# jonassibbesen/rpvg

Measured on AMD Instinct MI355X. Metric: read-pairs quantified/sec, higher is better.
Workload: dtype f64

## Files before the change

### rpvg_amd/csrc/subset_em.hip

```cpp

#include "common.hpp"
#include "subset_pack.hpp"

#include <cmath>
#include <memory>

using namespace rpvg_hip_detail;

namespace {

constexpr uint32_t kMaxSelected = 1024;

struct MergedList {
    const uint32_t * a;
    const uint32_t * b;
    uint32_t na, nb, i, j;
    __device__ __forceinline__ MergedList(const uint32_t * a_in, uint32_t na_in, const uint32_t * b_in, uint32_t nb_in)
        : a(a_in), b(b_in), na(na_in), nb(nb_in), i(0), j(0) {}
    __device__ __forceinline__ bool done() const { return i >= na && j >= nb; }
    __device__ __forceinline__ uint32_t next() {
        if (j >= nb || (i < na && a[i] <= b[j])) return a[i++];
        return b[j++];
    }
};

struct Columns {
    const uint64_t * group_path_off;
    const uint32_t * group_path;
    uint64_t first_column;
    __device__ __forceinline__ MergedList list(const uint32_t first, const uint32_t second) const {
        const uint64_t a0 = group_path_off[first_column + first], a1 = group_path_off[first_column + first + 1];
        const uint64_t b0 = group_path_off[first_column + second], b1 = group_path_off[first_column + second + 1];
        return MergedList(group_path + a0, static_cast<uint32_t>(a1 - a0), group_path + b0, static_cast<uint32_t>(b1 - b0));
    }
};

__device__ __forceinline__ int compareLists(MergedList x, MergedList y) {
    while (!x.done() && !y.done()) {
        const uint32_t px = x.next(), py = y.next();
        if (px != py) return px < py ? -1 : 1;
    }
    if (x.done() && y.done()) return 0;
    return x.done() ? -1 : 1;
}

struct SelectArgs {
    uint32_t num_matrices;
    const uint32_t * pair_count;
    const uint64_t * pair_cap_off;
    const uint32_t * pair_first;
    const uint32_t * pair_second;
    const double * pair_value;
    const uint64_t * group_off;
    const uint64_t * group_path_off;
    const uint32_t * group_path;
    const uint32_t * cluster;
    const uint64_t * mat_rows;
    const uint64_t * cluster_row_off;
    const uint64_t * row_ent_off;
    const uint64_t * slot_off;
    double min_hap_prob;
    uint32_t segment_rows;
    uint32_t * slot_first;
    uint32_t * slot_second;
    double * slot_weight;
    uint32_t * slot_length;
    uint32_t * slot_columns;
    MatrixTotals * totals;
    SubsetHeader * header;
    uint32_t * big_matrices;
};

constexpr uint32_t kSmallSelected = 64;
constexpr uint32_t kSmallCachedPaths = 1024, kWideCachedPaths = 6144;

struct CachedColumns {
    const uint64_t * group_path_off;
    const uint32_t * paths;
    uint64_t first_column, base;
    __device__ __forceinline__ MergedList list(const uint32_t first, const uint32_t second) const {
        const uint64_t a0 = group_path_off[first_column + first], a1 = group_path_off[first_column + first + 1];
        const uint64_t b0 = group_path_off[first_column + second], b1 = group_path_off[first_column + second + 1];
        return MergedList(paths + (a0 - base), static_cast<uint32_t>(a1 - a0), paths + (b0 - base), static_cast<uint32_t>(b1 - b0));
    }
};

template <uint32_t CAP, uint32_t CACHE, int BLOCK>
__device__ __forceinline__ void selectSubsetsOfMatrix(const SelectArgs & args, const uint32_t m) {
    __shared__ uint32_t sel[CAP];
    __shared__ unsigned long long hash[CAP];
    __shared__ uint32_t length[CAP];
    __shared__ uint32_t leader[CAP];
    __shared__ double weight[CAP];
    __shared__ uint32_t order[CAP];
    __shared__ uint32_t cached_paths[CACHE];
    __shared__ uint32_t scratch[BLOCK / 64];
    __shared__ double sum_posterior;
    __shared__ unsigned long long red[3];
    __shared__ uint32_t n_retained;
    const uint32_t n_pairs = args.pair_count[m];
    const uint64_t base = args.pair_cap_off[m];
    const uint32_t * first = args.pair_first + base;
    const uint32_t * second = args.pair_second + base;
    const double * value = args.pair_value + base;
    const uint32_t k = args.cluster[m];
    MatrixTotals * out_totals = args.totals + m;
    const uint64_t col0 = args.group_off[m], col1 = args.group_off[m + 1];
    const uint64_t path0 = args.group_path_off[col0], path1 = args.group_path_off[col1];
    const bool cached = path1 - path0 <= CACHE;
    if (cached) {
        for (uint32_t i = threadIdx.x; i < path1 - path0; i += BLOCK) cached_paths[i] = args.group_path[path0 + i];
    }
    const CachedColumns columns{args.group_path_off, cached ? cached_paths : args.group_path, col0, cached ? path0 : 0};

    uint32_t n_sel = 0;
    for (uint32_t c = 0; c < n_pairs; c += BLOCK) {
        const uint32_t i = c + threadIdx.x;
        const uint32_t take = (i < n_pairs && value[i] >= args.min_hap_prob) ? 1u : 0u;
        uint32_t total;
        const uint32_t at = n_sel + blockExclusiveScan<BLOCK>(take, total, scratch);
        if (take && at < CAP) sel[at] = i;
        n_sel += total;
    }
    if (n_sel > CAP) {
        if (threadIdx.x == 0) {
            atomicAdd(&args.header->select_overflow, 1ull);
            *out_totals = MatrixTotals{0, 0, 0, 0, 0, 0};
        }
        return;
    }
    __syncthreads();
    if (threadIdx.x == 0) {
        double sum = 0;
        for (uint32_t s = 0; s < n_sel; ++s) sum += value[sel[s]];
        sum_posterior = sum;
        red[0] = red[1] = red[2] = 0;
        n_retained = 0;
    }
    for (uint32_t s = threadIdx.x; s < n_sel; s += BLOCK) {
        MergedList list = columns.list(first[sel[s]], second[sel[s]]);
        unsigned long long h = 1469598103934665603ull;
        uint32_t n = 0;
        while (!list.done()) {
            h = (h ^ list.next()) * 1099511628211ull;
            ++n;
        }
        hash[s] = h;
        length[s] = n;
    }
    __syncthreads();
    for (uint32_t s = threadIdx.x; s < n_sel; s += BLOCK) {
        uint32_t lead = s;
        for (uint32_t t = 0; t < s; ++t) {
            if (hash[t] == hash[s] && length[t] == length[s] &&
                compareLists(columns.list(first[sel[t]], second[sel[t]]), columns.list(first[sel[s]], second[sel[s]])) == 0) {
                lead = t;
                break;
            }
        }
        leader[s] = lead;
    }
    __syncthreads();
    for (uint32_t s = threadIdx.x; s < n_sel; s += BLOCK) {
        double w = 0;
        if (leader[s] == s) {
            for (uint32_t t = s; t < n_sel; ++t) {
                if (leader[t] == s) w += value[sel[t]];
            }
            w /= sum_posterior;
            if (w >= args.min_hap_prob) order[atomicAdd(&n_retained, 1u)] = s;
        }
        weight[s] = w;
    }
    __syncthreads();
    const uint32_t n_ret = n_retained;
    uint32_t padded = 1;
    while (padded < n_ret) padded <<= 1;
    for (uint32_t i = n_ret + threadIdx.x; i < padded; i += BLOCK) order[i] = 0xffffffffu;
    __syncthreads();
    auto before = [&](const uint32_t x, const uint32_t y) {
        if (x == 0xffffffffu) return false;
        if (y == 0xffffffffu) return true;
        return compareLists(columns.list(first[sel[x]], second[sel[x]]), columns.list(first[sel[y]], second[sel[y]])) < 0;
    };
    for (uint32_t size = 2; size <= padded; size <<= 1) {
        for (uint32_t stride = size >> 1; stride > 0; stride >>= 1) {
            for (uint32_t i = threadIdx.x; i < padded; i += BLOCK) {
                const uint32_t partner = i ^ stride;
                if (partner > i) {
                    const bool ascending = (i & size) == 0;
                    const uint32_t x = order[i], y = order[partner];
                    if (before(y, x) == ascending) {
                        order[i] = y;
                        order[partner] = x;
                    }
                }
            }
            __syncthreads();
        }
    }
    const uint64_t slot0 = args.slot_off[m];
    unsigned long long my_subsets = 0, my_length = 0, my_columns = 0;
    for (uint32_t rank = threadIdx.x; rank < n_ret; rank += BLOCK) {
        const uint32_t s = order[rank];
        uint32_t distinct = 0, previous = 0xffffffffu;
        MergedList walk = columns.list(first[sel[s]], second[sel[s]]);
        while (!walk.done()) {
            const uint32_t path = walk.next();
            distinct += (path != previous) ? 1u : 0u;
            previous = path;
        }
        args.slot_first[slot0 + rank] = first[sel[s]];
        args.slot_second[slot0 + rank] = second[sel[s]];
        args.slot_weight[slot0 + rank] = weight[s];
        args.slot_length[slot0 + rank] = length[s];
        args.slot_columns[slot0 + rank] = distinct;
        my_subsets += 1;
        my_length += length[s];
        my_columns += distinct;
    }
    if (my_subsets) {
        atomicAdd(&red[0], my_subsets);
        atomicAdd(&red[1], my_length);
        atomicAdd(&red[2], my_columns);
    }
    __syncthreads();
    if (threadIdx.x == 0) {
        const uint64_t r0 = args.cluster_row_off[k], r1 = args.cluster_row_off[k + 1];
        const unsigned long long rows = r1 - r0, entries = args.row_ent_off[r1] - args.row_ent_off[r0];
        *out_totals = MatrixTotals{red[0], red[1], red[2], red[0] * rows, red[0] * entries, red[0] * ((rows + args.segment_rows - 1) / args.segment_rows)};
    }
}

__global__ __launch_bounds__(64) void subsetSelectSmallKernel(const SelectArgs args) {
    const uint32_t m = blockIdx.x;
    if (m >= args.num_matrices) return;
    if (args.pair_count[m] > kSmallSelected) {
        if (threadIdx.x == 0) args.big_matrices[atomicAdd(&args.header->big_count, 1u)] = m;
        return;
    }
    selectSubsetsOfMatrix<kSmallSelected, kSmallCachedPaths, 64>(args, m);
}

__global__ __launch_bounds__(256) void subsetSelectWideKernel(const SelectArgs args) {
    const uint32_t count = args.header->big_count;
    for (uint32_t item = blockIdx.x; item < count; item += gridDim.x) {
        selectSubsetsOfMatrix<kMaxSelected, kWideCachedPaths, 256>(args, args.big_matrices[item]);
        __syncthreads();
    }
}

struct ExpandArgs {
    uint32_t num_matrices;
    const SubsetHeader * header;
    const MatrixTotals * totals;
    const MatrixTotals * bases;
    const uint64_t * slot_off;
    const uint32_t * slot_first;
    const uint32_t * slot_second;
    const double * slot_weight;
    const uint32_t * slot_length;
    const uint32_t * slot_columns;
    const uint64_t * group_off;
    const uint64_t * group_path_off;
    const uint32_t * group_path;
    const uint32_t * cluster;
    const uint64_t * cluster_row_off;
    const uint64_t * row_ent_off;
    uint32_t * sub_cluster;
    double * sub_weight;
    uint64_t * path_off;
    uint32_t * path;
    uint64_t * col_off;
    uint32_t * col_path;
    uint64_t * row_base;
    uint64_t * ent_base;
    uint64_t * seg_first;
    uint32_t * item_problem;
    uint32_t segment_rows;
    uint64_t * subset_off;
};

__global__ __launch_bounds__(256) void subsetExpandKernel(const ExpandArgs args) {
    constexpr int BLOCK = 256;
    __shared__ uint32_t scratch[BLOCK / 64];
    const uint32_t m = blockIdx.x;
    if (m >= args.num_matrices) return;
    const MatrixTotals base = args.bases[m];
    if (threadIdx.x == 0) {
        args.subset_off[m] = args.header->overflow ? 0 : base.subsets;
        if (m + 1 == args.num_matrices) args.subset_off[m + 1] = args.header->overflow ? 0 : args.header->subsets;
    }
    if (args.header->overflow) return;
    const uint32_t n = static_cast<uint32_t>(args.totals[m].subsets);
    const uint64_t slot0 = args.slot_off[m];
    const Columns columns{args.group_path_off, args.group_path, args.group_off[m]};
    const uint32_t k = args.cluster[m];
    const uint64_t r0 = args.cluster_row_off[k], r1 = args.cluster_row_off[k + 1];
    const uint64_t rows = r1 - r0, entries = args.row_ent_off[r1] - args.row_ent_off[r0];
    uint64_t length_run = base.list_length, columns_run = base.columns;
    for (uint32_t c = 0; c < n; c += BLOCK) {
        const uint32_t r = c + threadIdx.x;
        const uint32_t len = r < n ? args.slot_length[slot0 + r] : 0u, cols = r < n ? args.slot_columns[slot0 + r] : 0u;
        uint32_t len_total, cols_total;
        const uint32_t len_before = blockExclusiveScan<BLOCK>(len, len_total, scratch);
        const uint32_t cols_before = blockExclusiveScan<BLOCK>(cols, cols_total, scratch);
        if (r < n) {
            const uint64_t s = base.subsets + r;
            const uint64_t p0 = length_run + len_before, c0 = columns_run + cols_before;
            args.sub_cluster[s] = k;
            args.sub_weight[s] = args.slot_weight[slot0 + r];
            args.path_off[s] = p0;
            args.col_off[s] = c0;
            args.row_base[s] = base.rows + static_cast<uint64_t>(r) * rows;
            args.ent_base[s] = base.entries + static_cast<uint64_t>(r) * entries;
            const uint64_t segments = (rows + args.segment_rows - 1) / args.segment_rows, item0 = base.segments + static_cast<uint64_t>(r) * segments;
            args.seg_first[s] = item0;
            for (uint64_t item = item0; item < item0 + segments; ++item) args.item_problem[item] = static_cast<uint32_t>(s);
            MergedList list = columns.list(args.slot_first[slot0 + r], args.slot_second[slot0 + r]);
            uint32_t previous = 0xffffffffu;
            uint64_t pw = p0, cw = c0;
            while (!list.done()) {
                const uint32_t path = list.next();
                args.path[pw++] = path;
                if (path != previous) args.col_path[cw++] = path;
                previous = path;
            }
        }
        length_run += len_total;
        columns_run += cols_total;
    }
}

constexpr uint32_t kMergeLdsRecords = 2048;
constexpr unsigned long long kMergeNoRecord = ~0ull;
constexpr uint32_t kMergePathBits = 27, kMergeRankBits = 10;

struct MergeArgs {
    const SubsetHeader * header;
    uint32_t num_matrices;
    const uint64_t * subset_off;
    const double * weight;
    const uint64_t * path_off;
    const uint32_t * path;
    const uint64_t * col_off;
    const uint32_t * col_path;
    const double * abundances;
    const double * noise;
    const double * total;
    const uint32_t * cluster;
    const uint64_t * cluster_path_off;
    const uint32_t * path_group_id;
    unsigned long long * sort_key;
    uint32_t * sort_pos;
    double * rec_a0;
    double * rec_a1;
    uint32_t * merge_bad;
    unsigned char * packed;
};

__global__ __launch_bounds__(256) void subsetMergeKernel(const MergeArgs args) {
    constexpr int BLOCK = 256;
    __shared__ unsigned long long s_key[kMergeLdsRecords];
    __shared__ uint32_t s_pos[kMergeLdsRecords];
    __shared__ uint32_t s_scan[BLOCK / 64];
    const SubsetHeader h = *args.header;
    if (h.overflow) return;
    const uint32_t m = blockIdx.x, tid = threadIdx.x;
    const uint64_t M = args.num_matrices;
    if (m >= M) return;
    const PackedLayout lay = packedLayout(M, h.subsets, h.list_length, h.columns);
    uint32_t * set_count = reinterpret_cast<uint32_t *>(args.packed + lay.set_count);
    double * cluster_noise = reinterpret_cast<double *>(args.packed + lay.cluster_noise);
    uint32_t * set_first = reinterpret_cast<uint32_t *>(args.packed + lay.set_first);
    uint32_t * set_second = reinterpret_cast<uint32_t *>(args.packed + lay.set_second);
    double * set_posterior = reinterpret_cast<double *>(args.packed + lay.set_posterior);
    double * set_abund = reinterpret_cast<double *>(args.packed + lay.set_abund);
    const uint64_t s0 = args.subset_off[m];
    const uint32_t n = static_cast<uint32_t>(args.subset_off[m + 1] - s0);
    if (n == 0) {
        if (tid == 0) {
            set_count[m] = 0;
            cluster_noise[m] = 0.0;
        }
        return;
    }
    const uint64_t base = args.path_off[s0];
    const uint32_t Lm = static_cast<uint32_t>(args.path_off[s0 + n] - base);
    const uint32_t * gid = args.path_group_id + args.cluster_path_off[args.cluster[m]];
    if (tid == BLOCK - 1) {
        double noise = 0.0, sum_hap_prob = 0.0;
        for (uint32_t r = 0; r < n; ++r) {
            const double w = args.weight[s0 + r];
            sum_hap_prob = addRounded(sum_hap_prob, w);
            noise = addRounded(noise, mulRounded(args.noise[s0 + r], w));
        }
        cluster_noise[m] = addRounded(noise, mulRounded(addRounded(1.0, -sum_hap_prob), args.total[s0]));
    }
    uint32_t P2 = 2;
    while (P2 < Lm) P2 <<= 1;
    unsigned long long * keys = s_key;
    uint32_t * order = s_pos;
    if (P2 > kMergeLdsRecords) {
        keys = args.sort_key + 2 * base;
        order = args.sort_pos + 2 * base;
    }
    for (uint32_t pos = tid; pos < P2; pos += BLOCK) {
        unsigned long long key = kMergeNoRecord;
        if (pos < Lm) {
            uint32_t lo = 0, hi = n - 1;
            while (lo < hi) {
                const uint32_t mid = (lo + hi + 1) >> 1;
                if (args.path_off[s0 + mid] - base <= pos) lo = mid; else hi = mid - 1;
            }
            const uint32_t r = lo;
            const uint32_t l0 = static_cast<uint32_t>(args.path_off[s0 + r] - base), L = static_cast<uint32_t>(args.path_off[s0 + r + 1] - base) - l0;
            const uint32_t * list = args.path + base + l0;
            const uint32_t j = pos - l0;
            const uint32_t g = gid[list[j]];
            uint32_t members = 0, first = 0, second = 0;
            for (uint32_t t = 0; t < L; ++t) {
                if (gid[list[t]] == g) {
                    if (members == 0) first = t;
                    else if (members == 1) second = t;
                    ++members;
                }
            }
            if (members > 2) *args.merge_bad = 1;
            if (first == j && members <= 2) {
                const uint32_t p0 = list[first], p1 = (members == 2) ? list[second] : 0xffffffffu;
                const double w = args.weight[s0 + r];
                const uint64_t c0 = args.col_off[s0 + r];
                const uint32_t C = static_cast<uint32_t>(args.col_off[s0 + r + 1] - c0);
                const uint32_t * cols = args.col_path + c0;
                auto column = [&](const uint32_t p) {
                    uint32_t a = 0, b = C;
                    while (a < b) {
                        const uint32_t mid = (a + b) >> 1;
                        if (cols[mid] < p) a = mid + 1; else b = mid;
                    }
                    return a;
                };
                const double multiplicity = (members == 2 && p0 == p1) ? 2.0 : 1.0;
                args.rec_a0[base + pos] = mulRounded(args.abundances[c0 + column(p0)], w) / multiplicity;
                args.rec_a1[base + pos] = (members == 2) ? mulRounded(args.abundances[c0 + column(p1)], w) / multiplicity : 0.0;
                key = (static_cast<unsigned long long>(p0 + 1) << (kMergePathBits + kMergeRankBits)) |
                      (static_cast<unsigned long long>(members == 2 ? p1 + 1 : 0u) << kMergeRankBits) | r;
            }
        }
        keys[pos] = key;
        order[pos] = pos;
    }
    __syncthreads();
    for (uint32_t k2 = 2; k2 <= P2; k2 <<= 1) {
        for (uint32_t j2 = k2 >> 1; j2 > 0; j2 >>= 1) {
            for (uint32_t i = tid; i < P2; i += BLOCK) {
                const uint32_t x = i ^ j2;
                if (x > i) {
                    const unsigned long long a = keys[i], b = keys[x];
                    if ((a > b) == ((i & k2) == 0)) {
                        keys[i] = b;
                        keys[x] = a;
                        const uint32_t oa = order[i];
                        order[i] = order[x];
                        order[x] = oa;
                    }
                }
            }
            __syncthreads();
        }
    }
    uint32_t Q = 0;
    for (uint32_t c0 = 0; c0 < Lm; c0 += BLOCK) {
        const uint32_t i = c0 + tid;
        const unsigned long long key = i < Lm ? keys[i] : kMergeNoRecord;
        const bool start = key != kMergeNoRecord && (i == 0 || (keys[i - 1] >> kMergeRankBits) != (key >> kMergeRankBits));
        uint32_t total;
        const uint32_t before = blockExclusiveSum<BLOCK>(start ? 1u : 0u, total, s_scan);
        if (start) {
            const unsigned long long set = key >> kMergeRankBits;
            double posterior = 0.0, a0 = 0.0, a1 = 0.0;
            for (uint32_t e = i; e < Lm && keys[e] != kMergeNoRecord && (keys[e] >> kMergeRankBits) == set; ++e) {
                const uint32_t r = static_cast<uint32_t>(keys[e] & ((1u << kMergeRankBits) - 1u)), pos = order[e];
                posterior = addRounded(posterior, args.weight[s0 + r]);
                a0 = addRounded(a0, args.rec_a0[base + pos]);
                a1 = addRounded(a1, args.rec_a1[base + pos]);
            }
            const uint64_t q = base + Q + before;
            const uint32_t second = static_cast<uint32_t>(set & ((1u << kMergePathBits) - 1u));
            set_first[q] = static_cast<uint32_t>(set >> kMergePathBits) - 1;
            set_second[q] = second ? second - 1 : 0xffffffffu;
            set_posterior[q] = posterior;
            set_abund[2 * q] = a0;
            set_abund[2 * q + 1] = a1;
        }
        Q += total;
    }
    if (tid == 0) set_count[m] = Q;
}

}


static int nestedSubsetEmAttempt(rpvg_hip_ctx * ctx, const rpvg_hip_batch * batch, const rpvg_hip_groups * groups,
                                 const uint32_t * column_counts, double min_rel_likelihood, double min_hap_prob,
                                 uint32_t max_em_its, double max_rel_em_conv, double collapse_precision,
                                 rpvg_hip_subset_em ** result_out, bool * did_not_fit, PairSearchWork & search, const bool second_attempt) {
    *did_not_fit = false;
    RPVG_REQUIRE(min_rel_likelihood > 0, "rpvg_hip_nested_subset_em: min_rel_likelihood must be positive");
    RPVG_REQUIRE(max_em_its > 0, "rpvg_hip_nested_subset_em: max_em_its must be positive");
    RPVG_REQUIRE(groups->batch == batch, "rpvg_hip_nested_subset_em: the matrices were built on another batch");
    const uint32_t M = groups->num_matrices;
    RPVG_REQUIRE(M == 0 || column_counts || groups->d_column_counts, "rpvg_hip_nested_subset_em: column_counts is NULL");
    std::unique_ptr<rpvg_hip_subset_em> res(new (std::nothrow) rpvg_hip_subset_em());
    if (!res) {
        setError("rpvg_hip_nested_subset_em: out of host memory");
        return RPVG_HIP_ERR_ALLOC;
    }
    res->num_matrices = M;

    const bool disabled = std::getenv("RPVG_HIP_NO_DEVICE_SUBSETS") != nullptr;
    if (disabled || !(min_hap_prob * kMaxSelected >= 1.0)) {
        setError("rpvg_hip_nested_subset_em: not taken (min_hap_prob %g admits more than %u subsets per cluster, or RPVG_HIP_NO_DEVICE_SUBSETS)",
                 min_hap_prob, kMaxSelected);
        return RPVG_HIP_ERR_UNSUPPORTED;
    }
    std::unique_ptr<HostScope> scope(new HostScope("subset em: bounds"));
    uint64_t slots = 0, lane_rows = 0, lane_entries = 0, lane_paths = 0, max_cluster_work = 0;
    uint32_t max_paths = 0;
    std::vector<uint64_t> slot_off(M + 1, 0);
    for (uint32_t m = 0; m < M; ++m) {
        const uint64_t G = groups->h_num_cols[m];
        slot_off[m + 1] = slot_off[m] + std::min<uint64_t>(G * (G + 1) / 2, kMaxSelected);
        const uint32_t k = groups->h_cluster[m];
        lane_rows += batch->h_cluster_row_off[k + 1] - batch->h_cluster_row_off[k];
        lane_entries += batch->h_cluster_ent_off[k + 1] - batch->h_cluster_ent_off[k];
        lane_paths += groups->h_num_paths[m];
        max_paths = std::max(max_paths, groups->h_num_paths[m]);
        max_cluster_work = std::max<uint64_t>(max_cluster_work, (batch->h_cluster_row_off[k + 1] - batch->h_cluster_row_off[k]) +
                                                                    (batch->h_cluster_ent_off[k + 1] - batch->h_cluster_ent_off[k]));
    }
    slots = slot_off[M];
    if (M > 0 && 8ull * (5ull * (static_cast<uint64_t>(max_paths) + 1) + 6) > 156 * 1024) {
        setError("rpvg_hip_nested_subset_em: not taken (a cluster with %u paths: EM vectors in global memory)", max_paths);
        return RPVG_HIP_ERR_UNSUPPORTED;
    }

    std::lock_guard<std::mutex> lock(ctx->mutex);
    RPVG_HIP_CHECK(hipSetDevice(ctx->device));
    hipStream_t st = ctx->stream;
    if (M == 0) {
        *result_out = res.release();
        return RPVG_HIP_OK;
    }
    SubsetEmHints & hints = ctx->subset_hints;
    auto planned = [](const double per_unit, const unsigned long long units, const double headroom) {
        return static_cast<unsigned long long>(std::ceil(per_unit * headroom * static_cast<double>(units)));
    };
    unsigned long long cap_subsets = std::min<unsigned long long>(slots, hints.subsets_per_matrix > 0 ? planned(hints.subsets_per_matrix, M, 1.25) + 256 : std::max<unsigned long long>(8ull * M, 16384));
    unsigned long long cap_length = std::max<unsigned long long>(planned(hints.list_per_path, lane_paths, 2.0), std::max<unsigned long long>(8 * lane_paths, 1u << 20));
    unsigned long long cap_rows = hints.rows_per_row > 0 ? planned(hints.rows_per_row, lane_rows, 1.25) + 65536 : 8 * lane_rows;
    unsigned long long cap_entries = hints.entries_per_entry > 0 ? planned(hints.entries_per_entry, lane_entries, 1.25) + 65536 : 8 * lane_entries;
    if (hints.retry) {
        cap_subsets = std::min<unsigned long long>(slots, std::max(cap_subsets, hints.retry_subsets + 64));
        cap_length = std::max(cap_length, hints.retry_list_length + 64);
        cap_rows = std::max(cap_rows, hints.retry_rows + 64);
        cap_entries = std::max(cap_entries, hints.retry_entries + 64);
        hints.retry = false;
    }
    const unsigned long long cap_columns = cap_length;
    const unsigned long long cap_items = cap_rows / emFillSegmentRows() + cap_subsets;

    scope.reset(new HostScope("subset em: search + kernels queued"));
    const size_t header_room = 256;
    int rc = RPVG_HIP_OK;
    if (!second_attempt) {
        search.extra_u64 = slot_off.data();
        search.extra_u64_count = M + 1;
        search.extra_zero_bytes = header_room + emQueuesBytes();
        rc = queuePairSearch(ctx, groups, column_counts, min_rel_likelihood, search);
        if (rc != RPVG_HIP_OK) return rc;
    } else {
        const hipError_t zeroed = zeroAsync(search.d_extra_zero.ptr, search.extra_zero_bytes, st);
        if (zeroed != hipSuccess) {
            setError("rpvg_hip_nested_subset_em: %s", hipGetErrorString(zeroed));
            return RPVG_HIP_ERR_RUNTIME;
        }
    }

    hipError_t e = hipSuccess;
    auto ok = [&](hipError_t r) { if (e == hipSuccess) e = r; return e == hipSuccess; };
    const uint64_t * d_slot_off = search.d_extra_u64.ptr;
    SubsetHeader * header = reinterpret_cast<SubsetHeader *>(search.d_extra_zero.ptr);
    static_assert(sizeof(SubsetHeader) <= 256, "room for the header");
    DeviceBuffer<uint32_t> d_slot_first, d_slot_second, d_slot_length, d_slot_columns;
    DeviceBuffer<double> d_slot_weight;
    DeviceBuffer<unsigned char> d_totals, d_bases, d_packed;
    ok(d_slot_first.alloc(slots));
    ok(d_slot_second.alloc(slots));
    ok(d_slot_length.alloc(slots));
    ok(d_slot_columns.alloc(slots));
    ok(d_slot_weight.alloc(slots));
    ok(d_totals.alloc(sizeof(MatrixTotals) * M));
    ok(d_bases.alloc(sizeof(MatrixTotals) * M));
    DeviceBuffer<uint32_t> d_big_matrices;
    ok(d_big_matrices.alloc(M));
    DeviceBuffer<uint32_t> d_sub_cluster, d_path, d_col_path, d_iters, d_kept_rows, d_kept_entries;
    DeviceBuffer<double> d_sub_weight, d_abund, d_noise, d_total;
    DeviceBuffer<uint64_t> d_path_off, d_col_off, d_row_base, d_ent_base, d_subset_off, d_seg_first;
    DeviceBuffer<uint32_t> d_item_problem;
    ok(d_sub_cluster.alloc(cap_subsets));
    ok(d_sub_weight.alloc(cap_subsets));
    ok(d_path_off.alloc(cap_subsets + 1));
    ok(d_col_off.alloc(cap_subsets + 1));
    ok(d_row_base.alloc(cap_subsets));
    ok(d_ent_base.alloc(cap_subsets));
    ok(d_subset_off.alloc(M + 1));
    ok(d_seg_first.alloc(cap_subsets + 1));
    ok(d_item_problem.alloc(cap_items));
    ok(d_path.alloc(cap_length));
    ok(d_col_path.alloc(cap_columns));
    ok(d_abund.alloc(cap_columns));
    ok(d_noise.alloc(cap_subsets));
    ok(d_total.alloc(cap_subsets));
    ok(d_iters.alloc(cap_subsets));
    ok(d_kept_rows.alloc(cap_subsets));
    ok(d_kept_entries.alloc(cap_subsets));
    const size_t packed_capacity = packedLayout(M, cap_subsets, cap_length, cap_columns).bytes;
    ok(d_packed.alloc(packed_capacity));
    const bool merge_here = batch->path_group_id.ptr != nullptr && max_paths < (1u << kMergePathBits) - 2;
    DeviceBuffer<unsigned long long> d_merge_key;
    DeviceBuffer<uint32_t> d_merge_pos;
    DeviceBuffer<double> d_merge_a0, d_merge_a1;
    if (merge_here) {
        ok(d_merge_key.alloc(2 * cap_length + 2));
        ok(d_merge_pos.alloc(2 * cap_length + 2));
        ok(d_merge_a0.alloc(cap_length));
        ok(d_merge_a1.alloc(cap_length));
    }
    void * pinned_header = nullptr;
    if (e == hipSuccess && pinnedAlloc(&pinned_header, sizeof(SubsetHeader)) != hipSuccess) e = hipErrorOutOfMemory;
    hipEvent_t header_here = nullptr;
    if (e == hipSuccess) ok(hipEventCreateWithFlags(&header_here, hipEventDisableTiming));
    if (e != hipSuccess) {
        setError("rpvg_hip_nested_subset_em: %s", hipGetErrorString(e));
        (void) hipStreamSynchronize(st);
        leavePairSearch(ctx);
        if (pinned_header) pinnedFree(pinned_header);
        if (header_here) (void) hipEventDestroy(header_here);
        return (e == hipErrorOutOfMemory) ? RPVG_HIP_ERR_ALLOC : RPVG_HIP_ERR_RUNTIME;
    }
    MatrixTotals * totals = reinterpret_cast<MatrixTotals *>(d_totals.ptr);
    MatrixTotals * bases = reinterpret_cast<MatrixTotals *>(d_bases.ptr);

    std::unique_ptr<HostScope> part_scope(new HostScope("subset em: select + offsets + expand queued"));
    int span = ctx->spanBegin(FAM_BUILD);
    SelectArgs sa;
    sa.num_matrices = M;
    sa.pair_count = search.d_tail.ptr;
    sa.pair_cap_off = search.d_pair_cap_off.ptr;
    sa.pair_first = search.d_out_first.ptr;
    sa.pair_second = search.d_out_second.ptr;
    sa.pair_value = search.d_out_value.ptr;
    sa.group_off = groups->d_group_off;
    sa.group_path_off = groups->d_group_path_off;
    sa.group_path = groups->d_group_path;
    sa.cluster = groups->d_cluster;
    sa.mat_rows = groups->mat_rows.ptr;
    sa.cluster_row_off = batch->cluster_row_off.ptr;
    sa.row_ent_off = batch->row_ent_off.ptr;
    sa.slot_off = d_slot_off;
    sa.min_hap_prob = min_hap_prob;
    sa.segment_rows = emFillSegmentRows();
    sa.slot_first = d_slot_first.ptr;
    sa.slot_second = d_slot_second.ptr;
    sa.slot_weight = d_slot_weight.ptr;
    sa.slot_length = d_slot_length.ptr;
    sa.slot_columns = d_slot_columns.ptr;
    sa.totals = totals;
    sa.header = header;
    sa.big_matrices = d_big_matrices.ptr;
    subsetSelectSmallKernel<<<dim3(M), dim3(64), 0, st>>>(sa);
    subsetSelectWideKernel<<<dim3(std::min<uint32_t>(M, 128)), dim3(256), 0, st>>>(sa);
    const bool check_build = !groups->build_checked && groups->build_error_flag.ptr;
    OffsetsArgs oa;
    oa.pair_count = search.d_tail.ptr;
    oa.log_evals = reinterpret_cast<const unsigned long long *>(search.d_tail.ptr + search.evals_word);
    oa.build_error = check_build ? groups->build_error_flag.ptr : nullptr;
    oa.num_matrices = M;
    oa.totals = totals;
    oa.bases = bases;
    oa.header = header;
    oa.cap_subsets = cap_subsets;
    oa.cap_length = cap_length;
    oa.cap_columns = cap_columns;
    oa.cap_rows = cap_rows;
    oa.cap_entries = cap_entries;
    oa.cap_items = cap_items;
    oa.seg_first = d_seg_first.ptr;
    oa.path_off = d_path_off.ptr;
    oa.col_off = d_col_off.ptr;
    subsetOffsetsKernel<<<dim3(1), dim3(1024), 0, st>>>(oa);
    SubsetHeader * h_header = static_cast<SubsetHeader *>(pinned_header);
    ok(hipMemcpyAsync(h_header, header, sizeof(SubsetHeader), hipMemcpyDeviceToHost, st));
    ok(hipEventRecord(header_here, st));
    ExpandArgs ea;
    ea.num_matrices = M;
    ea.header = header;
    ea.totals = totals;
    ea.bases = bases;
    ea.slot_off = d_slot_off;
    ea.slot_first = d_slot_first.ptr;
    ea.slot_second = d_slot_second.ptr;
    ea.slot_weight = d_slot_weight.ptr;
    ea.slot_length = d_slot_length.ptr;
    ea.slot_columns = d_slot_columns.ptr;
    ea.group_off = groups->d_group_off;
    ea.group_path_off = groups->d_group_path_off;
    ea.group_path = groups->d_group_path;
    ea.cluster = groups->d_cluster;
    ea.cluster_row_off = batch->cluster_row_off.ptr;
    ea.row_ent_off = batch->row_ent_off.ptr;
    ea.sub_cluster = d_sub_cluster.ptr;
    ea.sub_weight = d_sub_weight.ptr;
    ea.path_off = d_path_off.ptr;
    ea.path = d_path.ptr;
    ea.col_off = d_col_off.ptr;
    ea.col_path = d_col_path.ptr;
    ea.row_base = d_row_base.ptr;
    ea.ent_base = d_ent_base.ptr;
    ea.seg_first = d_seg_first.ptr;
    ea.item_problem = d_item_problem.ptr;
    ea.segment_rows = emFillSegmentRows();
    ea.subset_off = d_subset_off.ptr;
    subsetExpandKernel<<<dim3(M), dim3(256), 0, st>>>(ea);
    ok(hipGetLastError());
    ctx->spanEnd(span);
    ctx->stats.build_launches += 4;
    leavePairSearch(ctx);

    part_scope.reset();
    EmProblemList list;
    list.P_bound = static_cast<uint32_t>(std::min<unsigned long long>(cap_subsets, 0xfffffffeull));
    list.d_num_problems = &header->num_problems;
    list.d_cluster = d_sub_cluster.ptr;
    list.d_col_off = d_col_off.ptr;
    list.d_col_path = d_col_path.ptr;
    list.d_row_base = d_row_base.ptr;
    list.d_ent_base = d_ent_base.ptr;
    list.rows_capacity = cap_rows;
    list.entries_capacity = cap_entries;
    list.d_seg_first = d_seg_first.ptr;
    list.d_item_problem = d_item_problem.ptr;
    list.items_bound = static_cast<uint32_t>(std::min<unsigned long long>(cap_items, 0xfffffffeull));
    list.d_num_items = &header->num_items;
    list.max_cols = max_paths + 1;
    list.max_cluster_paths = max_paths;
    list.max_cluster_work = max_cluster_work;
    list.wide_capacity = 0;
    EmOutputs out{d_abund.ptr, d_noise.ptr, d_iters.ptr, d_kept_rows.ptr, d_kept_entries.ptr, d_total.ptr};
    EmSolveWork work;
    work.zeroed_queues = search.d_extra_zero.ptr + header_room;
    if (e == hipSuccess) {
        rc = queueEmSolve(ctx, batch, list, max_em_its, max_rel_em_conv, out, work, collapse_precision);
        if (rc != RPVG_HIP_OK) {
            (void) hipStreamSynchronize(st);
            (void) hipEventDestroy(header_here);
            pinnedFree(pinned_header);
            return rc;
        }
    }
    part_scope.reset(new HostScope("subset em: merge + pack queued"));
    static_assert(sizeof(SubsetHeader) <= 192, "the merge's flag word sits behind the header");
    uint32_t * d_merge_bad = reinterpret_cast<uint32_t *>(search.d_extra_zero.ptr + 192);
    if (merge_here && e == hipSuccess) {
        MergeArgs ma;
        ma.header = header;
        ma.num_matrices = M;
        ma.subset_off = d_subset_off.ptr;
        ma.weight = d_sub_weight.ptr;
        ma.path_off = d_path_off.ptr;
        ma.path = d_path.ptr;
        ma.col_off = d_col_off.ptr;
        ma.col_path = d_col_path.ptr;
        ma.abundances = d_abund.ptr;
        ma.noise = d_noise.ptr;
        ma.total = d_total.ptr;
        ma.cluster = groups->d_cluster;
        ma.cluster_path_off = batch->cluster_path_off.ptr;
        ma.path_group_id = batch->path_group_id.ptr;
        ma.sort_key = d_merge_key.ptr;
        ma.sort_pos = d_merge_pos.ptr;
        ma.rec_a0 = d_merge_a0.ptr;
        ma.rec_a1 = d_merge_a1.ptr;
        ma.merge_bad = d_merge_bad;
        ma.packed = d_packed.ptr;
        const int merge_span = ctx->spanBegin(FAM_BUILD);
        subsetMergeKernel<<<dim3(M), dim3(256), 0, st>>>(ma);
        ctx->spanEnd(merge_span);
        ctx->stats.build_launches += 1;
    }
    PackArgs pa;
    pa.merge_bad = merge_here ? d_merge_bad : nullptr;
    pa.header = header;
    pa.num_matrices = M;
    pa.subset_off = d_subset_off.ptr;
    pa.weight = d_sub_weight.ptr;
    pa.path_off = d_path_off.ptr;
    pa.col_off = d_col_off.ptr;
    pa.abundances = d_abund.ptr;
    pa.noise = d_noise.ptr;
    pa.total = d_total.ptr;
    pa.path = d_path.ptr;
    pa.col_path = d_col_path.ptr;
    pa.iterations = d_iters.ptr;
    pa.kept_rows = d_kept_rows.ptr;
    pa.kept_entries = d_kept_entries.ptr;
    pa.packed = d_packed.ptr;
    packResultsKernel<<<dim3(256), dim3(256), 0, st>>>(pa);
    ok(hipGetLastError());

    part_scope.reset();
    scope.reset(new HostScope("subset em: header"));
    if (e == hipSuccess) ok(waitEvent(header_here));
    (void) hipEventDestroy(header_here);
    if (e != hipSuccess) {
        setError("rpvg_hip_nested_subset_em: %s", hipGetErrorString(e));
        (void) hipStreamSynchronize(st);
        pinnedFree(pinned_header);
        return (e == hipErrorOutOfMemory) ? RPVG_HIP_ERR_ALLOC : RPVG_HIP_ERR_RUNTIME;
    }
    const SubsetHeader got = *h_header;
    pinnedFree(pinned_header);
    {
        auto fold = [](double & kept, const unsigned long long needed, const unsigned long long units) {
            kept = std::max(0.9 * kept, static_cast<double>(needed) / static_cast<double>(std::max<unsigned long long>(units, 1)));
        };
        fold(hints.subsets_per_matrix, got.subsets, M);
        fold(hints.list_per_path, got.list_length, lane_paths);
        fold(hints.rows_per_row, got.rows, lane_rows);
        fold(hints.entries_per_entry, got.entries, lane_entries);
    }
    if (got.build_bad) {
        (void) hipStreamSynchronize(st);
        setError(got.build_bad == 2 ? "rpvg_hip_groups_build: a group lists a path twice" : "rpvg_hip_groups_build: a group refers to a path outside its cluster");
        return RPVG_HIP_ERR_INVALID;
    }
    groups->build_checked = true;
    if (got.overflow) {
        (void) hipStreamSynchronize(st);
        setError("rpvg_hip_nested_subset_em: not taken (%llu subsets, %llu rows, %llu entries, %llu selected-diplotype overflows: over the reserved "
                 "capacity)", got.subsets, got.rows, got.entries, got.select_overflow);
        if (!got.select_overflow) {
            hints.retry = true;
            hints.retry_subsets = got.subsets;
            hints.retry_list_length = std::max(got.list_length, got.columns);
            hints.retry_rows = got.rows;
            hints.retry_entries = got.entries;
            *did_not_fit = true;
        }
        return RPVG_HIP_ERR_UNSUPPORTED;
    }
    scope.reset(new HostScope("subset em: wait for the EM + download"));
    const uint64_t S = got.subsets;
    const PackedLayout lay = packedLayout(M, S, got.list_length, got.columns);
    if (pinnedAlloc(&res->block, std::max<size_t>(lay.bytes, 64)) != hipSuccess) {
        (void) hipStreamSynchronize(st);
        setError("rpvg_hip_nested_subset_em: out of page-locked host memory");
        return RPVG_HIP_ERR_ALLOC;
    }
    unsigned char * host = static_cast<unsigned char *>(res->block);
    ok(hipMemcpyAsync(host, d_packed.ptr, lay.bytes, hipMemcpyDeviceToHost, st));
    ok(waitStream(st));
    if (e != hipSuccess) {
        setError("rpvg_hip_nested_subset_em: %s", hipGetErrorString(e));
        return RPVG_HIP_ERR_RUNTIME;
    }
    accountPairSearch(ctx, groups, search, got.log_evals, got.kept_pairs);

    rpvg_hip_subset_em_view & v = res->view;
    v.num_matrices = M;
    v.subset_off = reinterpret_cast<const uint64_t *>(host + lay.subset_off);
    v.weight = reinterpret_cast<const double *>(host + lay.weight);
    v.path_off = reinterpret_cast<const uint64_t *>(host + lay.path_off);
    v.path = reinterpret_cast<const uint32_t *>(host + lay.path);
    v.col_off = reinterpret_cast<const uint64_t *>(host + lay.col_off);
    v.col_path = reinterpret_cast<const uint32_t *>(host + lay.col_path);
    v.abundances = reinterpret_cast<const double *>(host + lay.abundances);
    v.noise_count = reinterpret_cast<const double *>(host + lay.noise);
    v.total_count = reinterpret_cast<const double *>(host + lay.total);
    v.iterations = reinterpret_cast<const uint32_t *>(host + lay.iterations);
    if (merge_here) {
        if (*reinterpret_cast<const uint32_t *>(host + lay.merge_flags)) {
            setError("rpvg_hip_nested_subset_em: a diplotype's path subset holds more than two paths of one transcript (PathInfo::group_id): "
                     "the reference asserts against it (src/path_abundance_estimator.cpp:722)");
            return RPVG_HIP_ERR_INVALID;
        }
        v.set_count = reinterpret_cast<const uint32_t *>(host + lay.set_count);
        v.cluster_noise_count = reinterpret_cast<const double *>(host + lay.cluster_noise);
        v.set_first = reinterpret_cast<const uint32_t *>(host + lay.set_first);
        v.set_second = reinterpret_cast<const uint32_t *>(host + lay.set_second);
        v.set_posterior = reinterpret_cast<const double *>(host + lay.set_posterior);
        v.set_abundance = reinterpret_cast<const double *>(host + lay.set_abund);
    }
    res->num_subsets = S;
    accountEmSolve(ctx, static_cast<uint32_t>(S), v.col_off, reinterpret_cast<const uint32_t *>(host + lay.kept_rows),
                   reinterpret_cast<const uint32_t *>(host + lay.kept_entries), v.iterations);
    *result_out = res.release();
    return RPVG_HIP_OK;
}

extern "C" int rpvg_hip_nested_subset_em(rpvg_hip_ctx * ctx, const rpvg_hip_batch * batch, const rpvg_hip_groups * groups,
                                         const uint32_t * column_counts, double min_rel_likelihood, double min_hap_prob,
                                         uint32_t max_em_its, double max_rel_em_conv, double collapse_precision,
                                         rpvg_hip_subset_em ** result_out) {
    RPVG_REQUIRE(ctx && batch && groups && result_out, "rpvg_hip_nested_subset_em: NULL argument");
    *result_out = nullptr;
    bool did_not_fit = false;
    PairSearchWork search;
    int rc = nestedSubsetEmAttempt(ctx, batch, groups, column_counts, min_rel_likelihood, min_hap_prob, max_em_its, max_rel_em_conv, collapse_precision,
                                   result_out, &did_not_fit, search, false);
    if (rc == RPVG_HIP_ERR_UNSUPPORTED && did_not_fit) {
        static const bool trace = std::getenv("RPVG_AMD_TRACE") != nullptr;
        if (trace) std::fprintf(stderr, "[rpvg_hip trace]   subset em: second attempt (%s)\n", rpvg_hip_last_error());
        rc = nestedSubsetEmAttempt(ctx, batch, groups, column_counts, min_rel_likelihood, min_hap_prob, max_em_its, max_rel_em_conv, collapse_precision,
                                   result_out, &did_not_fit, search, true);
    }
    return rc;
}

extern "C" int rpvg_hip_subset_em_get(const rpvg_hip_subset_em * result, rpvg_hip_subset_em_view * view_out) {
    RPVG_REQUIRE(result && view_out, "rpvg_hip_subset_em_get: NULL argument");
    *view_out = result->view;
    view_out->num_matrices = result->num_matrices;
    return RPVG_HIP_OK;
}

extern "C" void rpvg_hip_subset_em_free(rpvg_hip_subset_em * result) { delete result; }
```

Before: 2.526 billion.

## Replace quadratic subset dedup with hash-sorted grouping and packed sort keys

Subset selection now stages per-pair list offsets, lengths, hashes and distinct counts in LDS in one pass. It replaces the O(n^2) leader search with a bitonic sort by (hash, length), a segmented max-scan to find run heads, and comparisons only within runs. The final lexicographic sort compares packed 64-bit prefix keys and falls back to a full list compare only on ties. Wide-kernel LDS moves to a dynamic shared-memory struct, which adds LDS pressure and more barriers.

```diff
diff --git a/rpvg_amd/csrc/subset_em.hip b/rpvg_amd/csrc/subset_em.hip
--- a/rpvg_amd/csrc/subset_em.hip
+++ b/rpvg_amd/csrc/subset_em.hip
@@ -1,6 +1,7 @@
 
 #include "common.hpp"
 #include "subset_pack.hpp"
+#include "subset_select_plan.hpp"
 
 #include <cmath>
 #include <memory>
@@ -74,30 +75,57 @@
 constexpr uint32_t kSmallSelected = 64;
 constexpr uint32_t kSmallCachedPaths = 1024, kWideCachedPaths = 6144;
 
-struct CachedColumns {
-    const uint64_t * group_path_off;
+template <uint32_t CAP, uint32_t CACHE>
+struct SelectLds {
+    union {
+        unsigned long long hash[CAP];
+        double weight[CAP];
+    };
+    union {
+        double value[CAP];
+        unsigned long long key[CAP];
+    };
+    uint32_t sel[CAP];
+    uint32_t a_off[CAP], b_off[CAP];
+    uint32_t b_len[CAP], length[CAP];
+    uint32_t distinct[CAP];
+    uint32_t sorted[CAP];
+    uint32_t head[CAP];
+    uint32_t leader[CAP];
+    uint32_t order[CAP];
+    uint32_t cached_paths[CACHE];
+    unsigned long long red[3];
+    double sum_posterior;
+    uint32_t scratch[4];
+    uint32_t n_retained;
+    uint32_t max_path;
+};
+constexpr size_t kWideSelectLds = sizeof(SelectLds<kMaxSelected, kWideCachedPaths>);
+
+struct StagedLists {
     const uint32_t * paths;
-    uint64_t first_column, base;
-    __device__ __forceinline__ MergedList list(const uint32_t first, const uint32_t second) const {
-        const uint64_t a0 = group_path_off[first_column + first], a1 = group_path_off[first_column + first + 1];
-        const uint64_t b0 = group_path_off[first_column + second], b1 = group_path_off[first_column + second + 1];
-        return MergedList(paths + (a0 - base), static_cast<uint32_t>(a1 - a0), paths + (b0 - base), static_cast<uint32_t>(b1 - b0));
+    const uint32_t * a_off;
+    const uint32_t * b_off;
+    const uint32_t * b_len;
+    const uint32_t * length;
+    __device__ __forceinline__ MergedList list(const uint32_t s) const {
+        return MergedList(paths + a_off[s], length[s] - b_len[s], paths + b_off[s], b_len[s]);
     }
 };
 
+template <int BLOCK, class Before>
+__device__ __forceinline__ void sortIndices(uint32_t * order, const uint32_t padded, Before before) {
+    for (uint32_t size = 2; size <= padded; size <<= 1) {
+        for (uint32_t stride = size >> 1; stride > 0; stride >>= 1) {
+            for (uint32_t p = threadIdx.x; p < rpvg_select::sortStagePairs(padded); p += BLOCK) rpvg_select::compareExchange(order, p, size, stride, before);
+            __syncthreads();
+        }
+    }
+}
+
 template <uint32_t CAP, uint32_t CACHE, int BLOCK>
-__device__ __forceinline__ void selectSubsetsOfMatrix(const SelectArgs & args, const uint32_t m) {
-    __shared__ uint32_t sel[CAP];
-    __shared__ unsigned long long hash[CAP];
-    __shared__ uint32_t length[CAP];
-    __shared__ uint32_t leader[CAP];
-    __shared__ double weight[CAP];
-    __shared__ uint32_t order[CAP];
-    __shared__ uint32_t cached_paths[CACHE];
-    __shared__ uint32_t scratch[BLOCK / 64];
-    __shared__ double sum_posterior;
-    __shared__ unsigned long long red[3];
-    __shared__ uint32_t n_retained;
+__device__ __forceinline__ void selectSubsetsOfMatrix(const SelectArgs & args, const uint32_t m, SelectLds<CAP, CACHE> & lds) {
+    constexpr uint32_t ITEMS = (CAP + BLOCK - 1) / BLOCK;
     const uint32_t n_pairs = args.pair_count[m];
     const uint64_t base = args.pair_cap_off[m];
     const uint32_t * first = args.pair_first + base;
@@ -108,18 +136,24 @@
     const uint64_t col0 = args.group_off[m], col1 = args.group_off[m + 1];
     const uint64_t path0 = args.group_path_off[col0], path1 = args.group_path_off[col1];
     const bool cached = path1 - path0 <= CACHE;
-    if (cached) {
-        for (uint32_t i = threadIdx.x; i < path1 - path0; i += BLOCK) cached_paths[i] = args.group_path[path0 + i];
-    }
-    const CachedColumns columns{args.group_path_off, cached ? cached_paths : args.group_path, col0, cached ? path0 : 0};
+    if (threadIdx.x == 0) lds.max_path = 0;
+    __syncthreads();
+    uint32_t my_max_path = 0;
+    for (uint64_t i = threadIdx.x; i < path1 - path0; i += BLOCK) {
+        const uint32_t path = args.group_path[path0 + i];
+        if (cached) lds.cached_paths[i] = path;
+        my_max_path = path > my_max_path ? path : my_max_path;
+    }
+    if (my_max_path) atomicMax(&lds.max_path, my_max_path);
+    const StagedLists lists{cached ? lds.cached_paths : args.group_path + path0, lds.a_off, lds.b_off, lds.b_len, lds.length};
 
     uint32_t n_sel = 0;
     for (uint32_t c = 0; c < n_pairs; c += BLOCK) {
         const uint32_t i = c + threadIdx.x;
         const uint32_t take = (i < n_pairs && value[i] >= args.min_hap_prob) ? 1u : 0u;
         uint32_t total;
-        const uint32_t at = n_sel + blockExclusiveScan<BLOCK>(take, total, scratch);
-        if (take && at < CAP) sel[at] = i;
+        const uint32_t at = n_sel + blockExclusiveScan<BLOCK>(take, total, lds.scratch);
+        if (take && at < CAP) lds.sel[at] = i;
         n_sel += total;
     }
     if (n_sel > CAP) {
@@ -130,122 +164,169 @@
         return;
     }
     __syncthreads();
+    const uint32_t padded_sel = rpvg_select::paddedSize(n_sel);
+    {
+        uint32_t pair[ITEMS] = {}, col_a[ITEMS] = {}, col_b[ITEMS] = {};
+        uint64_t a0[ITEMS] = {}, a1[ITEMS] = {}, b0[ITEMS] = {}, b1[ITEMS] = {};
+#pragma unroll
+        for (uint32_t e = 0; e < ITEMS; ++e) {
+            const uint32_t s = threadIdx.x + e * BLOCK;
+            pair[e] = s < n_sel ? lds.sel[s] : 0u;
+        }
+#pragma unroll
+        for (uint32_t e = 0; e < ITEMS; ++e) {
+            const uint32_t s = threadIdx.x + e * BLOCK;
+            if (s < n_sel) {
+                lds.value[s] = value[pair[e]];
+                col_a[e] = first[pair[e]];
+                col_b[e] = second[pair[e]];
+            }
+        }
+#pragma unroll
+        for (uint32_t e = 0; e < ITEMS; ++e) {
+            const uint32_t s = threadIdx.x + e * BLOCK;
+            if (s < n_sel) {
+                a0[e] = args.group_path_off[col0 + col_a[e]];
+                a1[e] = args.group_path_off[col0 + col_a[e] + 1];
+                b0[e] = args.group_path_off[col0 + col_b[e]];
+                b1[e] = args.group_path_off[col0 + col_b[e] + 1];
+            }
+        }
+#pragma unroll
+        for (uint32_t e = 0; e < ITEMS; ++e) {
+            const uint32_t s = threadIdx.x + e * BLOCK;
+            if (s >= n_sel) {
+                if (s < padded_sel) lds.sorted[s] = rpvg_select::kPadding;
+                continue;
+            }
+            lds.a_off[s] = static_cast<uint32_t>(a0[e] - path0);
+            lds.b_off[s] = static_cast<uint32_t>(b0[e] - path0);
+            lds.b_len[s] = static_cast<uint32_t>(b1[e] - b0[e]);
+            lds.length[s] = static_cast<uint32_t>(a1[e] - a0[e]) + static_cast<uint32_t>(b1[e] - b0[e]);
+            MergedList walk(lists.paths + (a0[e] - path0), static_cast<uint32_t>(a1[e] - a0[e]), lists.paths + (b0[e] - path0), static_cast<uint32_t>(b1[e] - b0[e]));
+            unsigned long long h = 1469598103934665603ull;
+            uint32_t distinct = 0, previous = 0xffffffffu;
+            while (!walk.done()) {
+                const uint32_t path = walk.next();
+                h = (h ^ path) * 1099511628211ull;
+                distinct += (path != previous) ? 1u : 0u;
+                previous = path;
+            }
+            lds.hash[s] = h;
+            lds.distinct[s] = distinct;
+            lds.sorted[s] = s;
+        }
+    }
+    __syncthreads();
     if (threadIdx.x == 0) {
         double sum = 0;
-        for (uint32_t s = 0; s < n_sel; ++s) sum += value[sel[s]];
-        sum_posterior = sum;
-        red[0] = red[1] = red[2] = 0;
-        n_retained = 0;
-    }
-    for (uint32_t s = threadIdx.x; s < n_sel; s += BLOCK) {
-        MergedList list = columns.list(first[sel[s]], second[sel[s]]);
-        unsigned long long h = 1469598103934665603ull;
-        uint32_t n = 0;
-        while (!list.done()) {
-            h = (h ^ list.next()) * 1099511628211ull;
-            ++n;
-        }
-        hash[s] = h;
-        length[s] = n;
-    }
+        uint32_t s = 0;
+        for (; s + 8 <= n_sel; s += 8) {
+            double v[8];
+#pragma unroll
+            for (uint32_t j = 0; j < 8; ++j) v[j] = lds.value[s + j];
+#pragma unroll
+            for (uint32_t j = 0; j < 8; ++j) sum += v[j];
+        }
+        for (; s < n_sel; ++s) sum += lds.value[s];
+        lds.sum_posterior = sum;
+        lds.red[0] = lds.red[1] = lds.red[2] = 0;
+        lds.n_retained = 0;
+    }
+    sortIndices<BLOCK>(lds.sorted, padded_sel, [&](const uint32_t x, const uint32_t y) { return rpvg_select::groupBefore(lds.hash, lds.length, x, y); });
+    for (uint32_t p = threadIdx.x; p < n_sel; p += BLOCK) lds.head[p] = rpvg_select::isRunHead(lds.sorted, lds.hash, lds.length, p) ? p : 0u;
     __syncthreads();
-    for (uint32_t s = threadIdx.x; s < n_sel; s += BLOCK) {
-        uint32_t lead = s;
-        for (uint32_t t = 0; t < s; ++t) {
-            if (hash[t] == hash[s] && length[t] == length[s] &&
-                compareLists(columns.list(first[sel[t]], second[sel[t]]), columns.list(first[sel[s]], second[sel[s]])) == 0) {
-                lead = t;
-                break;
-            }
-        }
-        leader[s] = lead;
+    for (uint32_t d = 1; d < n_sel; d <<= 1) {
+        uint32_t next[ITEMS];
+#pragma unroll
+        for (uint32_t e = 0; e < ITEMS; ++e) {
+            const uint32_t p = threadIdx.x + e * BLOCK;
+            next[e] = p < n_sel ? rpvg_select::scanStep(lds.head, p, d) : 0u;
+        }
+        __syncthreads();
+#pragma unroll
+        for (uint32_t e = 0; e < ITEMS; ++e) {
+            const uint32_t p = threadIdx.x + e * BLOCK;
+            if (p < n_sel) lds.head[p] = next[e];
+        }
+        __syncthreads();
+    }
+    for (uint32_t p = threadIdx.x; p < n_sel; p += BLOCK) {
+        lds.leader[lds.sorted[p]] = rpvg_select::leaderAt(lds.sorted, lds.head, p, [&](const uint32_t t, const uint32_t s) { return compareLists(lists.list(t), lists.list(s)) == 0; });
     }
     __syncthreads();
-    for (uint32_t s = threadIdx.x; s < n_sel; s += BLOCK) {
-        double w = 0;
-        if (leader[s] == s) {
-            for (uint32_t t = s; t < n_sel; ++t) {
-                if (leader[t] == s) w += value[sel[t]];
-            }
-            w /= sum_posterior;
-            if (w >= args.min_hap_prob) order[atomicAdd(&n_retained, 1u)] = s;
-        }
-        weight[s] = w;
+    for (uint32_t p = threadIdx.x; p < n_sel; p += BLOCK) {
+        const uint32_t s = lds.sorted[p];
+        if (lds.leader[s] != s) continue;
+        const double w = rpvg_select::memberSum(lds.sorted, lds.head, lds.leader, lds.value, p, n_sel) / lds.sum_posterior;
+        lds.weight[s] = w;
+        if (w >= args.min_hap_prob) lds.order[atomicAdd(&lds.n_retained, 1u)] = s;
     }
     __syncthreads();
-    const uint32_t n_ret = n_retained;
-    uint32_t padded = 1;
-    while (padded < n_ret) padded <<= 1;
-    for (uint32_t i = n_ret + threadIdx.x; i < padded; i += BLOCK) order[i] = 0xffffffffu;
+    const uint32_t n_ret = lds.n_retained;
+    const uint32_t padded_ret = rpvg_select::paddedSize(n_ret);
+    const uint32_t key_bits = rpvg_select::keyElementBits(lds.max_path), key_elements = rpvg_select::keyElements(key_bits);
+    for (uint32_t r = threadIdx.x; r < padded_ret; r += BLOCK) {
+        if (r >= n_ret) {
+            lds.order[r] = rpvg_select::kPadding;
+            continue;
+        }
+        const uint32_t s = lds.order[r];
+        MergedList walk = lists.list(s);
+        unsigned long long key = 0;
+        for (uint32_t i = 0; i < key_elements; ++i) {
+            const bool present = !walk.done();
+            key = rpvg_select::keyAppend(key, key_bits, present, present ? walk.next() : 0u);
+        }
+        lds.key[s] = key;
+    }
     __syncthreads();
-    auto before = [&](const uint32_t x, const uint32_t y) {
-        if (x == 0xffffffffu) return false;
-        if (y == 0xffffffffu) return true;
-        return compareLists(columns.list(first[sel[x]], second[sel[x]]), columns.list(first[sel[y]], second[sel[y]])) < 0;
-    };
-    for (uint32_t size = 2; size <= padded; size <<= 1) {
-        for (uint32_t stride = size >> 1; stride > 0; stride >>= 1) {
-            for (uint32_t i = threadIdx.x; i < padded; i += BLOCK) {
-                const uint32_t partner = i ^ stride;
-                if (partner > i) {
-                    const bool ascending = (i & size) == 0;
-                    const uint32_t x = order[i], y = order[partner];
-                    if (before(y, x) == ascending) {
-                        order[i] = y;
-                        order[partner] = x;
-                    }
-                }
-            }
-            __syncthreads();
-        }
-    }
+    sortIndices<BLOCK>(lds.order, padded_ret, [&](const uint32_t x, const uint32_t y) {
+        return rpvg_select::rankBefore(lds.key, x, y, [&](const uint32_t u, const uint32_t v) { return compareLists(lists.list(u), lists.list(v)) < 0; });
+    });
     const uint64_t slot0 = args.slot_off[m];
     unsigned long long my_subsets = 0, my_length = 0, my_columns = 0;
     for (uint32_t rank = threadIdx.x; rank < n_ret; rank += BLOCK) {
-        const uint32_t s = order[rank];
-        uint32_t distinct = 0, previous = 0xffffffffu;
-        MergedList walk = columns.list(first[sel[s]], second[sel[s]]);
-        while (!walk.done()) {
-            const uint32_t path = walk.next();
-            distinct += (path != previous) ? 1u : 0u;
-            previous = path;
-        }
-        args.slot_first[slot0 + rank] = first[sel[s]];
-        args.slot_second[slot0 + rank] = second[sel[s]];
-        args.slot_weight[slot0 + rank] = weight[s];
-        args.slot_length[slot0 + rank] = length[s];
-        args.slot_columns[slot0 + rank] = distinct;
+        const uint32_t s = lds.order[rank];
+        args.slot_first[slot0 + rank] = first[lds.sel[s]];
+        args.slot_second[slot0 + rank] = second[lds.sel[s]];
+        args.slot_weight[slot0 + rank] = lds.weight[s];
+        args.slot_length[slot0 + rank] = lds.length[s];
+        args.slot_columns[slot0 + rank] = lds.distinct[s];
         my_subsets += 1;
-        my_length += length[s];
-        my_columns += distinct;
+        my_length += lds.length[s];
+        my_columns += lds.distinct[s];
     }
     if (my_subsets) {
-        atomicAdd(&red[0], my_subsets);
-        atomicAdd(&red[1], my_length);
-        atomicAdd(&red[2], my_columns);
+        atomicAdd(&lds.red[0], my_subsets);
+        atomicAdd(&lds.red[1], my_length);
+        atomicAdd(&lds.red[2], my_columns);
     }
     __syncthreads();
     if (threadIdx.x == 0) {
         const uint64_t r0 = args.cluster_row_off[k], r1 = args.cluster_row_off[k + 1];
         const unsigned long long rows = r1 - r0, entries = args.row_ent_off[r1] - args.row_ent_off[r0];
-        *out_totals = MatrixTotals{red[0], red[1], red[2], red[0] * rows, red[0] * entries, red[0] * ((rows + args.segment_rows - 1) / args.segment_rows)};
+        *out_totals = MatrixTotals{lds.red[0], lds.red[1], lds.red[2], lds.red[0] * rows, lds.red[0] * entries, lds.red[0] * ((rows + args.segment_rows - 1) / args.segment_rows)};
     }
 }
 
 __global__ __launch_bounds__(64) void subsetSelectSmallKernel(const SelectArgs args) {
+    __shared__ SelectLds<kSmallSelected, kSmallCachedPaths> lds;
     const uint32_t m = blockIdx.x;
     if (m >= args.num_matrices) return;
     if (args.pair_count[m] > kSmallSelected) {
         if (threadIdx.x == 0) args.big_matrices[atomicAdd(&args.header->big_count, 1u)] = m;
         return;
     }
-    selectSubsetsOfMatrix<kSmallSelected, kSmallCachedPaths, 64>(args, m);
+    selectSubsetsOfMatrix<kSmallSelected, kSmallCachedPaths, 64>(args, m, lds);
 }
 
 __global__ __launch_bounds__(256) void subsetSelectWideKernel(const SelectArgs args) {
+    extern __shared__ __align__(16) unsigned char wide_select_lds[];
+    SelectLds<kMaxSelected, kWideCachedPaths> & lds = *reinterpret_cast<SelectLds<kMaxSelected, kWideCachedPaths> *>(wide_select_lds);
     const uint32_t count = args.header->big_count;
     for (uint32_t item = blockIdx.x; item < count; item += gridDim.x) {
-        selectSubsetsOfMatrix<kMaxSelected, kWideCachedPaths, 256>(args, args.big_matrices[item]);
+        selectSubsetsOfMatrix<kMaxSelected, kWideCachedPaths, 256>(args, args.big_matrices[item], lds);
         __syncthreads();
     }
 }
@@ -681,7 +762,8 @@
     sa.header = header;
     sa.big_matrices = d_big_matrices.ptr;
     subsetSelectSmallKernel<<<dim3(M), dim3(64), 0, st>>>(sa);
-    subsetSelectWideKernel<<<dim3(std::min<uint32_t>(M, 128)), dim3(256), 0, st>>>(sa);
+    ok(hipFuncSetAttribute(reinterpret_cast<const void *>(&subsetSelectWideKernel), hipFuncAttributeMaxDynamicSharedMemorySize, static_cast<int>(kWideSelectLds)));
+    subsetSelectWideKernel<<<dim3(std::min<uint32_t>(M, 128)), dim3(256), kWideSelectLds, st>>>(sa);
     const bool check_build = !groups->build_checked && groups->build_error_flag.ptr;
     OffsetsArgs oa;
     oa.pair_count = search.d_tail.ptr;
diff --git a/rpvg_amd/csrc/subset_select_plan.hpp b/rpvg_amd/csrc/subset_select_plan.hpp
--- /dev/null
+++ b/rpvg_amd/csrc/subset_select_plan.hpp
@@ -0,0 +1,90 @@
+#ifndef RPVG_SUBSET_SELECT_PLAN_HPP
+#define RPVG_SUBSET_SELECT_PLAN_HPP
+
+#include <cstdint>
+
+#if defined(__HIPCC__)
+#define RPVG_SELECT_FN __host__ __device__ inline
+#else
+#define RPVG_SELECT_FN inline
+#endif
+
+namespace rpvg_select {
+
+constexpr uint32_t kPadding = 0xffffffffu;
+
+RPVG_SELECT_FN uint32_t paddedSize(const uint32_t n) {
+    uint32_t padded = 1;
+    while (padded < n) padded <<= 1;
+    return padded;
+}
+
+RPVG_SELECT_FN uint32_t sortStagePairs(const uint32_t padded) { return padded >> 1; }
+RPVG_SELECT_FN uint32_t pairLow(const uint32_t p, const uint32_t stride) { return ((p & ~(stride - 1)) << 1) | (p & (stride - 1)); }
+RPVG_SELECT_FN bool pairAscending(const uint32_t low, const uint32_t size) { return (low & size) == 0; }
+template <class Before>
+RPVG_SELECT_FN void compareExchange(uint32_t * order, const uint32_t p, const uint32_t size, const uint32_t stride, Before before) {
+    const uint32_t low = pairLow(p, stride), high = low | stride;
+    const uint32_t x = order[low], y = order[high];
+    if (before(y, x) == pairAscending(low, size)) {
+        order[low] = y;
+        order[high] = x;
+    }
+}
+
+RPVG_SELECT_FN bool groupBefore(const unsigned long long * hash, const uint32_t * length, const uint32_t x, const uint32_t y) {
+    if (x == kPadding || y == kPadding) return x != kPadding;
+    if (hash[x] != hash[y]) return hash[x] < hash[y];
+    if (length[x] != length[y]) return length[x] < length[y];
+    return x < y;
+}
+RPVG_SELECT_FN bool isRunHead(const uint32_t * sorted, const unsigned long long * hash, const uint32_t * length, const uint32_t p) {
+    if (p == 0) return true;
+    const uint32_t s = sorted[p], t = sorted[p - 1];
+    return hash[s] != hash[t] || length[s] != length[t];
+}
+RPVG_SELECT_FN uint32_t scanStep(const uint32_t * head, const uint32_t p, const uint32_t d) {
+    const uint32_t own = head[p];
+    if (p < d) return own;
+    const uint32_t other = head[p - d];
+    return other > own ? other : own;
+}
+template <class SameList>
+RPVG_SELECT_FN uint32_t leaderAt(const uint32_t * sorted, const uint32_t * head, const uint32_t p, SameList same_list) {
+    const uint32_t s = sorted[p];
+    for (uint32_t q = head[p]; q < p; ++q) {
+        if (same_list(sorted[q], s)) return sorted[q];
+    }
+    return s;
+}
+template <class Value>
+RPVG_SELECT_FN Value memberSum(const uint32_t * sorted, const uint32_t * head, const uint32_t * leader, const Value * value,
+                               const uint32_t p, const uint32_t n) {
+    const uint32_t s = sorted[p], h = head[p];
+    Value sum = 0;
+    for (uint32_t q = p; q < n && head[q] == h; ++q) {
+        const uint32_t t = sorted[q];
+        if (leader[t] == s) sum += value[t];
+    }
+    return sum;
+}
+
+RPVG_SELECT_FN uint32_t keyElementBits(const uint32_t max_path) {
+    uint32_t bits = 1;
+    while ((max_path + 1ull) >> bits) ++bits;
+    return bits;
+}
+RPVG_SELECT_FN uint32_t keyElements(const uint32_t bits) { return 64 / bits; }
+RPVG_SELECT_FN unsigned long long keyAppend(const unsigned long long key, const uint32_t bits, const bool present, const uint32_t e) {
+    return (key << bits) | (present ? e + 1ull : 0ull);
+}
+template <class ListBefore>
+RPVG_SELECT_FN bool rankBefore(const unsigned long long * key, const uint32_t x, const uint32_t y, ListBefore list_before) {
+    if (x == kPadding || y == kPadding) return x != kPadding;
+    if (key[x] != key[y]) return key[x] < key[y];
+    return list_before(x, y);
+}
+
+}
+
+#endif
```

New measurement: 2.558 billion, median of 6. 1.01x the previous value.
